# eridgd/WCT-TF

Hardware: AMD Instinct MI355X
Metric: stylized frames/sec @512x512, 5-level relu5->1 pipeline, alpha=0.8 (higher is better)
Workload: dtype f16

## Files before the change

### wct_tf_amd/csrc/conv_wino.hip

```cpp
#include "common.h"

namespace {
typedef unsigned int u32x4 __attribute__((ext_vector_type(4)));
typedef _Float16 h2 __attribute__((ext_vector_type(2)));
constexpr int TW = 16;
constexpr int PITCH = 20;
constexpr int BK = 32;

__device__ __forceinline__ half8 pk_sub(half8 a, half8 b) {
  u32x4 ua = __builtin_bit_cast(u32x4, a), ub = __builtin_bit_cast(u32x4, b), r;
#pragma unroll
  for (int i = 0; i < 4; ++i) {
    unsigned o;
    asm("v_pk_add_f16 %0, %1, %2 neg_lo:[0,1] neg_hi:[0,1]" : "=v"(o) : "v"(ua[i]), "v"(ub[i]));
    r[i] = o;
  }
  return __builtin_bit_cast(half8, r);
}

__device__ __forceinline__ int reflect_idx(int i, int n) {
  if (i < 0) i = -i;
  if (i >= n) i = 2 * n - 2 - i;
  i = i < 0 ? 0 : i;
  return i >= n ? n - 1 : i;
}

template <int TH, int BN, int WM, int WN, bool IL>
__global__ __launch_bounds__(256, TH >= 16 ? 1 : 2)
void conv3x3_wino_kernel(ConvArgs p, int tiles_x, int n_tiles) {
  constexpr int PR = TH / 2;
  constexpr int MT = (PR / 2) / WM;
  constexpr int NT = (BN / 32) / WN;
  constexpr int G = 256 / PR;
  constexpr int SL = (72 + G - 1) / G;
  constexpr int PATCH_BYTES = PR * 4 * PITCH * 64;
  constexpr int DUMP_OFF = 2 * PATCH_BYTES;
  constexpr int PF_TAP = 5;
  static_assert(PR % 2 == 0 && (PR / 2) % WM == 0 && 256 % PR == 0 && WM * WN == 4, "tile shape");

  extern __shared__ __attribute__((aligned(16))) unsigned char smem[];
  const int tid = threadIdx.x, lane = tid & 63, wave = tid >> 6;
  const int wm = wave / WN, wn = wave % WN;
  int bid = blockIdx.x;
  const int ntile = bid % n_tiles;
  bid /= n_tiles;
  const int tx = bid % tiles_x, ty = bid / tiles_x;
  const int b = blockIdx.y;
  const int y0 = ty * TH, x0 = tx * TW, n0 = ntile * BN;

  const int Hin = p.upsample ? p.H / 2 : p.H;
  const int Win = p.upsample ? p.W / 2 : p.W;
  const half_t* xb = p.x + (size_t)b * Hin * Win * p.Cin;
  const __amdgpu_buffer_rsrc_t w_rsrc = __builtin_amdgcn_make_buffer_rsrc((void*)p.w_wino, 0, 0x7FFFFFFF, 0x00020000);
  const __amdgpu_buffer_rsrc_t x_rsrc = __builtin_amdgcn_make_buffer_rsrc((void*)xb, 0, 0x7FFFFFFF, 0x00020000);

  const int lpr = tid / G, ls = tid % G;
  unsigned row_off[4], col_off[SL], dst_off[SL];
  bool slot_ok[SL];
#pragma unroll
  for (int i = 0; i < 4; ++i) {
    int iy = reflect_idx(y0 + 2 * lpr - 1 + i, p.H);
    if (p.upsample) iy >>= 1;
    row_off[i] = (unsigned)(iy * Win) * p.Cin * 2;
  }
#pragma unroll
  for (int j = 0; j < SL; ++j) {
    const int slot = ls + j * G;
    slot_ok[j] = slot < 72;
    const int px = slot_ok[j] ? slot >> 2 : 0, piece = slot & 3;
    int ix = reflect_idx(x0 - 1 + px, p.W);
    if (p.upsample) ix >>= 1;
    col_off[j] = (unsigned)(ix * p.Cin + piece * 8) * 2;
    dst_off[j] = ((lpr * 4 * PITCH + px) * 4 + (piece ^ ((px >> 2) & 3))) * 16;
    if (IL && !slot_ok[j]) dst_off[j] = DUMP_OFF + tid * 16;
  }
  u32x4 raw[SL][4];
  auto load_rows = [&](int chunk) {
#pragma unroll
    for (int j = 0; j < SL; ++j)
#pragma unroll
      for (int i = 0; i < 4; ++i)
        raw[j][i] = __builtin_amdgcn_raw_buffer_load_b128(x_rsrc, row_off[i] + col_off[j], chunk * BK * 2, 0);
  };
  auto park_rows = [&](int buf) {
#pragma unroll
    for (int j = 0; j < SL; ++j) {
      const half8 d0 = __builtin_bit_cast(half8, raw[j][0]), d1 = __builtin_bit_cast(half8, raw[j][1]);
      const half8 d2 = __builtin_bit_cast(half8, raw[j][2]), d3 = __builtin_bit_cast(half8, raw[j][3]);
      const half8 t0 = pk_sub(d0, d2), t1 = d1 + d2, t2 = pk_sub(d2, d1), t3 = pk_sub(d1, d3);
      if (slot_ok[j]) {
        unsigned char* d = smem + buf * PATCH_BYTES + dst_off[j];
        *reinterpret_cast<half8*>(d) = t0;
        *reinterpret_cast<half8*>(d + PITCH * 64) = t1;
        *reinterpret_cast<half8*>(d + 2 * PITCH * 64) = t2;
        *reinterpret_cast<half8*>(d + 3 * PITCH * 64) = t3;
      }
    }
  };

  const int frag_px = lane & 15, frag_pr = (lane & 31) >> 4, kgrp = lane >> 5;
  int rd_base[3][2];
#pragma unroll
  for (int kx = 0; kx < 3; ++kx)
#pragma unroll
    for (int ks = 0; ks < 2; ++ks) {
      const int px = frag_px + kx;
      rd_base[kx][ks] = (((wm * MT * 2 + frag_pr) * 4) * PITCH + px) * 64 + (((ks * 2 + kgrp) ^ ((px >> 2) & 3)) * 16);
    }
  const int c16 = p.Cin >> 4;
  unsigned wfrag[NT];
#pragma unroll
  for (int nt = 0; nt < NT; ++nt) wfrag[nt] = (((n0 >> 5) + wn * NT + nt) * 12 * c16 * 512 + lane * 8) * 2;

  f32x16 acc[4][NT][MT];
#pragma unroll
  for (int nt = 0; nt < NT; ++nt) {
    f32x4 bv[4];
#pragma unroll
    for (int rq = 0; rq < 4; ++rq) bv[rq] = *reinterpret_cast<const f32x4*>(p.bias + n0 + (wn * NT + nt) * 32 + 8 * rq + 4 * kgrp);
#pragma unroll
    for (int f = 0; f < 4; ++f)
#pragma unroll
      for (int mt = 0; mt < MT; ++mt)
#pragma unroll
        for (int r = 0; r < 16; ++r) acc[f][nt][mt][r] = f == 1 ? bv[r >> 2][r & 3] : 0.f;
  }

  const int n_chunks = p.Cin / BK;
  half8 wf[3][NT][2];
  half8 bf[IL ? 3 : 2][2][MT];
  auto load_w = [&](half8 (&dst)[NT][2], int tap12, int chunk) {
    const int soff = (tap12 * c16 + chunk * 2) * 1024;
#pragma unroll
    for (int nt = 0; nt < NT; ++nt)
#pragma unroll
      for (int ks = 0; ks < 2; ++ks)
        dst[nt][ks] = __builtin_bit_cast(half8, __builtin_amdgcn_raw_buffer_load_b128(w_rsrc, wfrag[nt] + ks * 1024, soff, 0));
  };
  auto read_b = [&](half8 (&dst)[2][MT], int f, int kx, int buf) {
#pragma unroll
    for (int ks = 0; ks < 2; ++ks)
#pragma unroll
      for (int mt = 0; mt < MT; ++mt)
        dst[ks][mt] = *reinterpret_cast<const half8*>(smem + buf * PATCH_BYTES + rd_base[kx][ks] + (mt * 8 + f) * PITCH * 64);
  };

  if constexpr (IL) {
    constexpr int NM = 2 * MT * NT;
    constexpr int NR = 2 * NT + 2 * MT;
#ifndef WINO_LT0
#define WINO_LT0 1
#define WINO_PT0 6
#endif
    constexpr int LT0 = WINO_LT0, PT0 = WINO_PT0;
    static_assert(LT0 + SL <= PT0 && PT0 + SL <= 10, "staging schedule");
#ifndef WINO_WRING
#define WINO_WRING 4
#endif
#ifndef WINO_ABL
#define WINO_ABL 0
#endif
#ifndef WINO_RAW_AUX
#define WINO_RAW_AUX 0
#endif
    constexpr int ABL = WINO_ABL;
    constexpr int WR = WINO_WRING, WA = WR - 1;
    static_assert(24 % WR == 0, "ring");
    half8 wq[WR][NT][2];
    half8 tq[4];
    load_rows(0);
#pragma unroll
    for (int i = 0; i < WA; ++i) load_w(wq[i], i, 0);
#pragma unroll
    for (int j = 0; j < SL; ++j) {
      const half8 d0 = __builtin_bit_cast(half8, raw[j][0]), d1 = __builtin_bit_cast(half8, raw[j][1]);
      const half8 d2 = __builtin_bit_cast(half8, raw[j][2]), d3 = __builtin_bit_cast(half8, raw[j][3]);
      unsigned char* d = smem + dst_off[j];
      *reinterpret_cast<half8*>(d) = pk_sub(d0, d2);
      *reinterpret_cast<half8*>(d + PITCH * 64) = d1 + d2;
      *reinterpret_cast<half8*>(d + 2 * PITCH * 64) = pk_sub(d2, d1);
      *reinterpret_cast<half8*>(d + 3 * PITCH * 64) = pk_sub(d1, d3);
    }
    asm volatile("s_waitcnt lgkmcnt(0)\n\ts_barrier" ::: "memory");
    read_b(bf[0], 0, 0, 0);
    read_b(bf[1], 0, 1, 0);
#pragma unroll 1
    for (int pair = 0; pair < n_chunks; pair += 2) {
#pragma unroll
      for (int t = 0; t < 24; ++t) {
        const int tt = t % 12, chunk_i = pair + t / 12, buf = t / 12;
        const int f = tt / 3, kx = tt % 3;
        const int chunk_n = chunk_i + 1 < n_chunks ? chunk_i + 1 : chunk_i;
        const int t3 = (tt + WA) % 12, c3 = tt + WA >= 12 ? chunk_n : chunk_i;
        const int t1 = (tt + 2) % 12, buf1 = tt >= 10 ? buf ^ 1 : buf;
        const int soff3 = (t3 * c16 + c3 * 2) * 1024;
#pragma unroll
        for (int j = 0; j < NM; ++j) {
          const int ks = j / (MT * NT), mt = (j / NT) % MT, nt = j % NT;
          if (!(ABL & 4)) acc[f][nt][mt] = __builtin_amdgcn_mfma_f32_32x32x16_f16(wq[t % WR][nt][ks], bf[t % 3][ks][mt], acc[f][nt][mt], 0, 0, 0);
          else asm volatile("" :: "v"(wq[t % WR][nt][ks]), "v"(bf[t % 3][ks][mt]));
#pragma unroll
          for (int k = j * NR / NM; k < (j + 1) * NR / NM; ++k) {
            if (k < 2 * NT) {
              if (!(ABL & 1)) wq[(t + WA) % WR][k / 2][k % 2] =
                  __builtin_bit_cast(half8, __builtin_amdgcn_raw_buffer_load_b128(w_rsrc, wfrag[k / 2] + (k % 2) * 1024, soff3, 0));
            } else {
              const int kk = k - 2 * NT, ks1 = kk / MT, mt1 = kk % MT;
              if (!(ABL & 8)) bf[(t + 2) % 3][ks1][mt1] = *reinterpret_cast<const half8*>(smem + buf1 * PATCH_BYTES + rd_base[t1 % 3][ks1] + (mt1 * 8 + t1 / 3) * PITCH * 64);
            }
          }
          if (tt >= LT0 && tt < LT0 + SL) {
            const int sl = tt - LT0;
            if (j < 4 && !(ABL & 2)) raw[sl][j] = __builtin_amdgcn_raw_buffer_load_b128(x_rsrc, (ABL & 64) ? (lane & 3) * 16 + j * 64 + sl * 256 : row_off[j] + col_off[sl], (ABL & 32) ? 0 : chunk_n * BK * 2, WINO_RAW_AUX);
          }
          if (tt >= PT0 && tt < PT0 + SL && !(ABL & 16)) {
            const int sl = tt - PT0;
            {
#pragma unroll
              for (int it = j * 8 / NM; it < (j + 1) * 8 / NM; ++it) {
                const int fq = it >> 1;
                if ((it & 1) == 0) {
                  const half8 da = __builtin_bit_cast(half8, raw[sl][fq == 0 ? 0 : fq == 1 ? 1 : fq == 2 ? 2 : 1]);
                  const half8 db = __builtin_bit_cast(half8, raw[sl][fq == 0 ? 2 : fq == 1 ? 2 : fq == 2 ? 1 : 3]);
                  tq[fq] = fq == 1 ? da + db : pk_sub(da, db);
                } else {
                  *reinterpret_cast<half8*>(smem + (buf ^ 1) * PATCH_BYTES * (slot_ok[sl] ? 1 : 0) + dst_off[sl] + fq * PITCH * 64) = tq[fq];
                }
              }
            }
          }
          __builtin_amdgcn_sched_barrier(0);
        }
        if (tt == 9) asm volatile("s_waitcnt lgkmcnt(0)\n\ts_barrier" ::: "memory");
      }
    }
  } else {
  load_rows(0);
  load_w(wf[0], 0, 0);
  load_w(wf[1], 1, 0);
  park_rows(0);
  asm volatile("s_waitcnt lgkmcnt(0)\n\ts_barrier" ::: "memory");
  read_b(bf[0], 0, 0, 0);

#pragma unroll 1
  for (int pair = 0; pair < n_chunks; pair += 2) {
#pragma unroll
    for (int t = 0; t < 24; ++t) {
      const int tt = t % 12, chunk_i = pair + t / 12, buf = t / 12;
      const int f = tt / 3, kx = tt % 3;
      const bool more = chunk_i + 1 < n_chunks;
      {
        const int t2 = (tt + 2) % 12;
        const int c2 = tt + 2 >= 12 ? (more ? chunk_i + 1 : chunk_i) : chunk_i;
        load_w(wf[(t + 2) % 3], t2, c2);
      }
      if (tt == PF_TAP && more) load_rows(chunk_i + 1);
      if (tt != 11) read_b(bf[(t + 1) & 1], (tt + 1) / 3, (tt + 1) % 3, buf);
      else if (more) read_b(bf[(t + 1) & 1], 0, 0, buf ^ 1);
      __builtin_amdgcn_sched_barrier(0);
#pragma unroll
      for (int ks = 0; ks < 2; ++ks)
#pragma unroll
        for (int mt = 0; mt < MT; ++mt)
#pragma unroll
          for (int nt = 0; nt < NT; ++nt)
            acc[f][nt][mt] = __builtin_amdgcn_mfma_f32_32x32x16_f16(wf[t % 3][nt][ks], bf[t & 1][ks][mt], acc[f][nt][mt], 0, 0, 0);
      __builtin_amdgcn_sched_barrier(0);
      if (tt == 10 && more) {
        park_rows(buf ^ 1);
        asm volatile("s_waitcnt lgkmcnt(0)\n\ts_barrier" ::: "memory");
      }
    }
  }

  }
  constexpr int OOB = (int)0x80000000u;
  const int Ho = p.pool ? (p.H + 1) / 2 : p.H, Wo = p.pool ? (p.W + 1) / 2 : p.W;
  const unsigned img_elems = (unsigned)Ho * Wo * p.Cout;
  const __amdgpu_buffer_rsrc_t r16 = __builtin_amdgcn_make_buffer_rsrc((void*)(p.y16 + (size_t)b * img_elems), 0, img_elems * 2, 0x00020000);
  const float lo1 = p.relu ? 0.f : -__builtin_inff();
  const h2 lo2 = {(half_t)lo1, (half_t)lo1};
  const h2 zero2 = {(half_t)0.f, (half_t)0.f};
  const int ox = x0 + frag_px;
  const int chan = n0 + wn * NT * 32;
#pragma unroll
  for (int mt = 0; mt < MT; ++mt) {
    const int oy = y0 + ((wm * MT + mt) * 2 + frag_pr) * 2;
    const bool in0 = (oy < p.H) & (ox < p.W), in1 = (oy + 1 < p.H) & (ox < p.W);
    int off[2];
    if (p.pool) {
      off[0] = in0 && (frag_px & 1) == 0 ? (((oy >> 1) * Wo + (ox >> 1)) * p.Cout + chan + 8 * kgrp) * 2 : OOB;
      off[1] = OOB;
    } else {
      off[0] = in0 ? ((oy * p.W + ox) * p.Cout + chan + 8 * kgrp) * 2 : OOB;
      off[1] = in1 ? (((oy + 1) * p.W + ox) * p.Cout + chan + 8 * kgrp) * 2 : OOB;
    }
#pragma unroll
    for (int nt = 0; nt < NT; ++nt) {
      unsigned pk[2][4][2];
#pragma unroll
      for (int rq = 0; rq < 4; ++rq) {
        f32x4 e, o;
#pragma unroll
        for (int j = 0; j < 4; ++j) {
          const int r = rq * 4 + j;
          const float m0 = acc[0][nt][mt][r], m1 = acc[1][nt][mt][r], m2 = acc[2][nt][mt][r], m3 = acc[3][nt][mt][r];
          e[j] = (m0 + m1) + m2;
          o[j] = (m1 - m2) - m3;
        }
        h2 e0 = {(half_t)e[0], (half_t)e[1]}, e1 = {(half_t)e[2], (half_t)e[3]};
        h2 o0 = {(half_t)o[0], (half_t)o[1]}, o1 = {(half_t)o[2], (half_t)o[3]};
        e0 = __builtin_elementwise_max(e0, lo2); e1 = __builtin_elementwise_max(e1, lo2);
        o0 = __builtin_elementwise_max(o0, lo2); o1 = __builtin_elementwise_max(o1, lo2);
        if (p.pool) {
          h2 q[2] = {__builtin_elementwise_max(in0 ? e0 : zero2, in1 ? o0 : zero2), __builtin_elementwise_max(in0 ? e1 : zero2, in1 ? o1 : zero2)};
#pragma unroll
          for (int d = 0; d < 2; ++d) {
            const unsigned tq = __builtin_bit_cast(unsigned, q[d]);
            const h2 nb = __builtin_bit_cast(h2, __builtin_amdgcn_update_dpp(0, (int)tq, 0xB1, 0xF, 0xF, true));
            q[d] = __builtin_elementwise_max(q[d], nb);
          }
          e0 = q[0]; e1 = q[1];
        }
        pk[0][rq][0] = __builtin_bit_cast(unsigned, e0); pk[0][rq][1] = __builtin_bit_cast(unsigned, e1);
        pk[1][rq][0] = __builtin_bit_cast(unsigned, o0); pk[1][rq][1] = __builtin_bit_cast(unsigned, o1);
      }
#pragma unroll
      for (int par = 0; par < 2; ++par) {
#pragma unroll
        for (int m = 0; m < 2; ++m) {
          auto sx = __builtin_amdgcn_permlane32_swap(pk[par][2 * m][0], pk[par][2 * m + 1][0], false, false);
          auto sy = __builtin_amdgcn_permlane32_swap(pk[par][2 * m][1], pk[par][2 * m + 1][1], false, false);
          u32x4 ov = {sx[0], sy[0], sx[1], sy[1]};
          __builtin_amdgcn_raw_buffer_store_b128(ov, r16, off[par] + (nt * 32 + 16 * m) * 2, 0, 0);
        }
      }
    }
  }
}

template <int TH, int BN, int WM, int WN, bool IL = false>
int launch_wino_cfg(const ConvArgs& a, hipStream_t s) {
  const int tiles_x = cdiv(a.W, TW), tiles_y = cdiv(a.H, TH), n_tiles = a.Cout / BN;
  const size_t lds = 2 * (size_t)(TH / 2) * 4 * PITCH * 64 + (IL ? 8192 : 0);
  HIP_TRY(hipFuncSetAttribute(reinterpret_cast<const void*>(&conv3x3_wino_kernel<TH, BN, WM, WN, IL>),
                              hipFuncAttributeMaxDynamicSharedMemorySize, (int)lds));
  hipLaunchKernelGGL((conv3x3_wino_kernel<TH, BN, WM, WN, IL>), dim3(tiles_x * tiles_y * n_tiles, a.B), dim3(256), lds, s, a, tiles_x, n_tiles);
  HIP_TRY(hipGetLastError());
  return WCT_OK;
}
}

bool conv3x3_wino_takes(const ConvArgs& a) {
  return a.w_wino != nullptr && a.y16 != nullptr && a.y32 == nullptr && a.usum == nullptr && a.img1 == nullptr &&
         a.Cin % 64 == 0 && a.Cout % 64 == 0 && (!a.pool || a.relu);
}

int launch_conv3x3_wino(const ConvArgs& a, hipStream_t s) {
  ARG_CHECK(conv3x3_wino_takes(a) && a.H > 1 && a.W > 1 && a.B > 0);
  ARG_CHECK(!a.upsample || (a.H % 2 == 0 && a.W % 2 == 0));
  ARG_CHECK((size_t)a.H * a.W * a.Cin * 2 < ((size_t)1 << 31));
  ARG_CHECK((size_t)a.H * a.W * a.Cout * 2 < ((size_t)1 << 31));
  const long px16 = (long)cdiv(a.W, TW) * cdiv(a.H, 16) * a.B;
  const long px8 = (long)cdiv(a.W, TW) * cdiv(a.H, 8) * a.B;
  if (a.Cout % 128 == 0 && px16 * (a.Cout / 128) >= 256) return launch_wino_cfg<16, 128, 1, 4, true>(a, s);
  if (a.Cout % 128 == 0 && px8 * (a.Cout / 128) >= 256) return launch_wino_cfg<8, 128, 1, 4>(a, s);
  return launch_wino_cfg<8, 64, 2, 2>(a, s);
}
```

Before: 684.2.

## Specialize Winograd conv for nearest-upsampled input to use three row transforms

Adds a compile-time UP variant of the Winograd F(2,3) conv kernel for inputs that were nearest-neighbour upsampled. Paired output rows then share duplicated source rows, so one input-transform row is zero and the kernel keeps only three transformed rows (9 taps instead of 12), with weight taps remapped. This cuts MFMA work, LDS footprint and input loads for the decoder's upsample convs. The cost is a rescheduled pipeline (ring size, staging taps) tuned only for the new tap count, and row clamping in place of reflection, which changes border semantics and relies on the tile start y0 being even.

New measurement: 685.3 (median of 6 runs). No clear change (+0.2%).

```diff
diff --git a/wct_tf_amd/csrc/conv_wino.hip b/wct_tf_amd/csrc/conv_wino.hip
--- a/wct_tf_amd/csrc/conv_wino.hip
+++ b/wct_tf_amd/csrc/conv_wino.hip
@@ -25,17 +25,20 @@
   return i >= n ? n - 1 : i;
 }
 
-template <int TH, int BN, int WM, int WN, bool IL>
+template <int TH, int BN, int WM, int WN, bool IL, bool UP>
 __global__ __launch_bounds__(256, TH >= 16 ? 1 : 2)
 void conv3x3_wino_kernel(ConvArgs p, int tiles_x, int n_tiles) {
+  constexpr int NF = UP ? 3 : 4;
+  constexpr int NTAP = NF * 3;
+  auto wtap = [](int t) { return (UP && t >= 6 ? t + 3 : t); };
   constexpr int PR = TH / 2;
   constexpr int MT = (PR / 2) / WM;
   constexpr int NT = (BN / 32) / WN;
   constexpr int G = 256 / PR;
   constexpr int SL = (72 + G - 1) / G;
-  constexpr int PATCH_BYTES = PR * 4 * PITCH * 64;
+  constexpr int PATCH_BYTES = PR * NF * PITCH * 64;
   constexpr int DUMP_OFF = 2 * PATCH_BYTES;
-  constexpr int PF_TAP = 5;
+  constexpr int PF_TAP = NTAP - 7;
   static_assert(PR % 2 == 0 && (PR / 2) % WM == 0 && 256 % PR == 0 && WM * WN == 4, "tile shape");
 
   extern __shared__ __attribute__((aligned(16))) unsigned char smem[];
@@ -48,19 +51,25 @@
   const int b = blockIdx.y;
   const int y0 = ty * TH, x0 = tx * TW, n0 = ntile * BN;
 
-  const int Hin = p.upsample ? p.H / 2 : p.H;
-  const int Win = p.upsample ? p.W / 2 : p.W;
+  const int Hin = UP ? p.H / 2 : p.H;
+  const int Win = UP ? p.W / 2 : p.W;
   const half_t* xb = p.x + (size_t)b * Hin * Win * p.Cin;
   const __amdgpu_buffer_rsrc_t w_rsrc = __builtin_amdgcn_make_buffer_rsrc((void*)p.w_wino, 0, 0x7FFFFFFF, 0x00020000);
   const __amdgpu_buffer_rsrc_t x_rsrc = __builtin_amdgcn_make_buffer_rsrc((void*)xb, 0, 0x7FFFFFFF, 0x00020000);
 
   const int lpr = tid / G, ls = tid % G;
-  unsigned row_off[4], col_off[SL], dst_off[SL];
+  unsigned row_off[NF], col_off[SL], dst_off[SL];
   bool slot_ok[SL];
 #pragma unroll
-  for (int i = 0; i < 4; ++i) {
-    int iy = reflect_idx(y0 + 2 * lpr - 1 + i, p.H);
-    if (p.upsample) iy >>= 1;
+  for (int i = 0; i < NF; ++i) {
+    int iy;
+    if constexpr (UP) {
+      iy = (y0 >> 1) + lpr - 1 + i;
+      iy = iy < 0 ? 0 : iy;
+      iy = iy >= Hin ? Hin - 1 : iy;
+    } else {
+      iy = reflect_idx(y0 + 2 * lpr - 1 + i, p.H);
+    }
     row_off[i] = (unsigned)(iy * Win) * p.Cin * 2;
   }
 #pragma unroll
@@ -69,31 +78,35 @@
     slot_ok[j] = slot < 72;
     const int px = slot_ok[j] ? slot >> 2 : 0, piece = slot & 3;
     int ix = reflect_idx(x0 - 1 + px, p.W);
-    if (p.upsample) ix >>= 1;
+    if (UP) ix >>= 1;
     col_off[j] = (unsigned)(ix * p.Cin + piece * 8) * 2;
-    dst_off[j] = ((lpr * 4 * PITCH + px) * 4 + (piece ^ ((px >> 2) & 3))) * 16;
+    dst_off[j] = ((lpr * NF * PITCH + px) * 4 + (piece ^ ((px >> 2) & 3))) * 16;
     if (IL && !slot_ok[j]) dst_off[j] = DUMP_OFF + tid * 16;
   }
-  u32x4 raw[SL][4];
+  u32x4 raw[SL][NF];
   auto load_rows = [&](int chunk) {
 #pragma unroll
     for (int j = 0; j < SL; ++j)
 #pragma unroll
-      for (int i = 0; i < 4; ++i)
+      for (int i = 0; i < NF; ++i)
         raw[j][i] = __builtin_amdgcn_raw_buffer_load_b128(x_rsrc, row_off[i] + col_off[j], chunk * BK * 2, 0);
   };
+  auto piece = [&](const u32x4 (&r)[NF], int q) {
+    const int ia = UP ? (q == 0 ? 0 : 1) : (q == 0 ? 0 : q == 1 ? 1 : q == 2 ? 2 : 1);
+    const int ib = UP ? (q == 0 ? 1 : q == 1 ? 1 : 2) : (q == 0 ? 2 : q == 1 ? 2 : q == 2 ? 1 : 3);
+    const half8 da = __builtin_bit_cast(half8, r[ia]), db = __builtin_bit_cast(half8, r[ib]);
+    return q == 1 ? da + db : pk_sub(da, db);
+  };
   auto park_rows = [&](int buf) {
 #pragma unroll
     for (int j = 0; j < SL; ++j) {
-      const half8 d0 = __builtin_bit_cast(half8, raw[j][0]), d1 = __builtin_bit_cast(half8, raw[j][1]);
-      const half8 d2 = __builtin_bit_cast(half8, raw[j][2]), d3 = __builtin_bit_cast(half8, raw[j][3]);
-      const half8 t0 = pk_sub(d0, d2), t1 = d1 + d2, t2 = pk_sub(d2, d1), t3 = pk_sub(d1, d3);
+      half8 t[NF];
+#pragma unroll
+      for (int q = 0; q < NF; ++q) t[q] = piece(raw[j], q);
       if (slot_ok[j]) {
         unsigned char* d = smem + buf * PATCH_BYTES + dst_off[j];
-        *reinterpret_cast<half8*>(d) = t0;
-        *reinterpret_cast<half8*>(d + PITCH * 64) = t1;
-        *reinterpret_cast<half8*>(d + 2 * PITCH * 64) = t2;
-        *reinterpret_cast<half8*>(d + 3 * PITCH * 64) = t3;
+#pragma unroll
+        for (int q = 0; q < NF; ++q) *reinterpret_cast<half8*>(d + q * PITCH * 64) = t[q];
       }
     }
   };
@@ -105,21 +118,21 @@
 #pragma unroll
     for (int ks = 0; ks < 2; ++ks) {
       const int px = frag_px + kx;
-      rd_base[kx][ks] = (((wm * MT * 2 + frag_pr) * 4) * PITCH + px) * 64 + (((ks * 2 + kgrp) ^ ((px >> 2) & 3)) * 16);
+      rd_base[kx][ks] = (((wm * MT * 2 + frag_pr) * NF) * PITCH + px) * 64 + (((ks * 2 + kgrp) ^ ((px >> 2) & 3)) * 16);
     }
   const int c16 = p.Cin >> 4;
   unsigned wfrag[NT];
 #pragma unroll
   for (int nt = 0; nt < NT; ++nt) wfrag[nt] = (((n0 >> 5) + wn * NT + nt) * 12 * c16 * 512 + lane * 8) * 2;
 
-  f32x16 acc[4][NT][MT];
+  f32x16 acc[NF][NT][MT];
 #pragma unroll
   for (int nt = 0; nt < NT; ++nt) {
     f32x4 bv[4];
 #pragma unroll
     for (int rq = 0; rq < 4; ++rq) bv[rq] = *reinterpret_cast<const f32x4*>(p.bias + n0 + (wn * NT + nt) * 32 + 8 * rq + 4 * kgrp);
 #pragma unroll
-    for (int f = 0; f < 4; ++f)
+    for (int f = 0; f < NF; ++f)
 #pragma unroll
       for (int mt = 0; mt < MT; ++mt)
 #pragma unroll
@@ -129,8 +142,8 @@
   const int n_chunks = p.Cin / BK;
   half8 wf[3][NT][2];
   half8 bf[IL ? 3 : 2][2][MT];
-  auto load_w = [&](half8 (&dst)[NT][2], int tap12, int chunk) {
-    const int soff = (tap12 * c16 + chunk * 2) * 1024;
+  auto load_w = [&](half8 (&dst)[NT][2], int tap, int chunk) {
+    const int soff = (wtap(tap) * c16 + chunk * 2) * 1024;
 #pragma unroll
     for (int nt = 0; nt < NT; ++nt)
 #pragma unroll
@@ -142,7 +155,7 @@
     for (int ks = 0; ks < 2; ++ks)
 #pragma unroll
       for (int mt = 0; mt < MT; ++mt)
-        dst[ks][mt] = *reinterpret_cast<const half8*>(smem + buf * PATCH_BYTES + rd_base[kx][ks] + (mt * 8 + f) * PITCH * 64);
+        dst[ks][mt] = *reinterpret_cast<const half8*>(smem + buf * PATCH_BYTES + rd_base[kx][ks] + (mt * 2 * NF + f) * PITCH * 64);
   };
 
   if constexpr (IL) {
@@ -152,8 +165,8 @@
 #define WINO_LT0 1
 #define WINO_PT0 6
 #endif
-    constexpr int LT0 = WINO_LT0, PT0 = WINO_PT0;
-    static_assert(LT0 + SL <= PT0 && PT0 + SL <= 10, "staging schedule");
+    constexpr int LT0 = UP ? 0 : WINO_LT0, PT0 = UP ? 4 : WINO_PT0;
+    static_assert(LT0 + SL <= PT0 && PT0 + SL <= NTAP - 2, "staging schedule");
 #ifndef WINO_WRING
 #define WINO_WRING 4
 #endif
@@ -164,22 +177,18 @@
 #define WINO_RAW_AUX 0
 #endif
     constexpr int ABL = WINO_ABL;
-    constexpr int WR = WINO_WRING, WA = WR - 1;
-    static_assert(24 % WR == 0, "ring");
+    constexpr int WR = UP ? 6 : WINO_WRING, WA = WR - 1;
+    static_assert((2 * NTAP) % WR == 0 && WA < NTAP, "ring");
     half8 wq[WR][NT][2];
-    half8 tq[4];
+    half8 tq[NF];
     load_rows(0);
 #pragma unroll
     for (int i = 0; i < WA; ++i) load_w(wq[i], i, 0);
 #pragma unroll
     for (int j = 0; j < SL; ++j) {
-      const half8 d0 = __builtin_bit_cast(half8, raw[j][0]), d1 = __builtin_bit_cast(half8, raw[j][1]);
-      const half8 d2 = __builtin_bit_cast(half8, raw[j][2]), d3 = __builtin_bit_cast(half8, raw[j][3]);
       unsigned char* d = smem + dst_off[j];
-      *reinterpret_cast<half8*>(d) = pk_sub(d0, d2);
-      *reinterpret_cast<half8*>(d + PITCH * 64) = d1 + d2;
-      *reinterpret_cast<half8*>(d + 2 * PITCH * 64) = pk_sub(d2, d1);
-      *reinterpret_cast<half8*>(d + 3 * PITCH * 64) = pk_sub(d1, d3);
+#pragma unroll
+      for (int q = 0; q < NF; ++q) *reinterpret_cast<half8*>(d + q * PITCH * 64) = piece(raw[j], q);
     }
     asm volatile("s_waitcnt lgkmcnt(0)\n\ts_barrier" ::: "memory");
     read_b(bf[0], 0, 0, 0);
@@ -187,13 +196,13 @@
 #pragma unroll 1
     for (int pair = 0; pair < n_chunks; pair += 2) {
 #pragma unroll
-      for (int t = 0; t < 24; ++t) {
-        const int tt = t % 12, chunk_i = pair + t / 12, buf = t / 12;
-        const int f = tt / 3, kx = tt % 3;
+      for (int t = 0; t < 2 * NTAP; ++t) {
+        const int tt = t % NTAP, chunk_i = pair + t / NTAP, buf = t / NTAP;
+        const int f = tt / 3;
         const int chunk_n = chunk_i + 1 < n_chunks ? chunk_i + 1 : chunk_i;
-        const int t3 = (tt + WA) % 12, c3 = tt + WA >= 12 ? chunk_n : chunk_i;
-        const int t1 = (tt + 2) % 12, buf1 = tt >= 10 ? buf ^ 1 : buf;
-        const int soff3 = (t3 * c16 + c3 * 2) * 1024;
+        const int t3 = (tt + WA) % NTAP, c3 = tt + WA >= NTAP ? chunk_n : chunk_i;
+        const int t1 = (tt + 2) % NTAP, buf1 = tt >= NTAP - 2 ? buf ^ 1 : buf;
+        const int soff3 = (wtap(t3) * c16 + c3 * 2) * 1024;
 #pragma unroll
         for (int j = 0; j < NM; ++j) {
           const int ks = j / (MT * NT), mt = (j / NT) % MT, nt = j % NT;
@@ -206,23 +215,21 @@
                   __builtin_bit_cast(half8, __builtin_amdgcn_raw_buffer_load_b128(w_rsrc, wfrag[k / 2] + (k % 2) * 1024, soff3, 0));
             } else {
               const int kk = k - 2 * NT, ks1 = kk / MT, mt1 = kk % MT;
-              if (!(ABL & 8)) bf[(t + 2) % 3][ks1][mt1] = *reinterpret_cast<const half8*>(smem + buf1 * PATCH_BYTES + rd_base[t1 % 3][ks1] + (mt1 * 8 + t1 / 3) * PITCH * 64);
+              if (!(ABL & 8)) bf[(t + 2) % 3][ks1][mt1] = *reinterpret_cast<const half8*>(smem + buf1 * PATCH_BYTES + rd_base[t1 % 3][ks1] + (mt1 * 2 * NF + t1 / 3) * PITCH * 64);
             }
           }
           if (tt >= LT0 && tt < LT0 + SL) {
             const int sl = tt - LT0;
-            if (j < 4 && !(ABL & 2)) raw[sl][j] = __builtin_amdgcn_raw_buffer_load_b128(x_rsrc, (ABL & 64) ? (lane & 3) * 16 + j * 64 + sl * 256 : row_off[j] + col_off[sl], (ABL & 32) ? 0 : chunk_n * BK * 2, WINO_RAW_AUX);
+            if (j < NF && !(ABL & 2)) raw[sl][j] = __builtin_amdgcn_raw_buffer_load_b128(x_rsrc, (ABL & 64) ? (lane & 3) * 16 + j * 64 + sl * 256 : row_off[j] + col_off[sl], (ABL & 32) ? 0 : chunk_n * BK * 2, WINO_RAW_AUX);
           }
           if (tt >= PT0 && tt < PT0 + SL && !(ABL & 16)) {
             const int sl = tt - PT0;
             {
 #pragma unroll
-              for (int it = j * 8 / NM; it < (j + 1) * 8 / NM; ++it) {
+              for (int it = j * 2 * NF / NM; it < (j + 1) * 2 * NF / NM; ++it) {
                 const int fq = it >> 1;
                 if ((it & 1) == 0) {
-                  const half8 da = __builtin_bit_cast(half8, raw[sl][fq == 0 ? 0 : fq == 1 ? 1 : fq == 2 ? 2 : 1]);
-                  const half8 db = __builtin_bit_cast(half8, raw[sl][fq == 0 ? 2 : fq == 1 ? 2 : fq == 2 ? 1 : 3]);
-                  tq[fq] = fq == 1 ? da + db : pk_sub(da, db);
+                  tq[fq] = piece(raw[sl], fq);
                 } else {
                   *reinterpret_cast<half8*>(smem + (buf ^ 1) * PATCH_BYTES * (slot_ok[sl] ? 1 : 0) + dst_off[sl] + fq * PITCH * 64) = tq[fq];
                 }
@@ -231,7 +238,7 @@
           }
           __builtin_amdgcn_sched_barrier(0);
         }
-        if (tt == 9) asm volatile("s_waitcnt lgkmcnt(0)\n\ts_barrier" ::: "memory");
+        if (tt == NTAP - 3) asm volatile("s_waitcnt lgkmcnt(0)\n\ts_barrier" ::: "memory");
       }
     }
   } else {
@@ -245,17 +252,17 @@
 #pragma unroll 1
   for (int pair = 0; pair < n_chunks; pair += 2) {
 #pragma unroll
-    for (int t = 0; t < 24; ++t) {
-      const int tt = t % 12, chunk_i = pair + t / 12, buf = t / 12;
-      const int f = tt / 3, kx = tt % 3;
+    for (int t = 0; t < 2 * NTAP; ++t) {
+      const int tt = t % NTAP, chunk_i = pair + t / NTAP, buf = t / NTAP;
+      const int f = tt / 3;
       const bool more = chunk_i + 1 < n_chunks;
       {
-        const int t2 = (tt + 2) % 12;
-        const int c2 = tt + 2 >= 12 ? (more ? chunk_i + 1 : chunk_i) : chunk_i;
+        const int t2 = (tt + 2) % NTAP;
+        const int c2 = tt + 2 >= NTAP ? (more ? chunk_i + 1 : chunk_i) : chunk_i;
         load_w(wf[(t + 2) % 3], t2, c2);
       }
       if (tt == PF_TAP && more) load_rows(chunk_i + 1);
-      if (tt != 11) read_b(bf[(t + 1) & 1], (tt + 1) / 3, (tt + 1) % 3, buf);
+      if (tt != NTAP - 1) read_b(bf[(t + 1) & 1], (tt + 1) / 3, (tt + 1) % 3, buf);
       else if (more) read_b(bf[(t + 1) & 1], 0, 0, buf ^ 1);
       __builtin_amdgcn_sched_barrier(0);
 #pragma unroll
@@ -266,7 +273,7 @@
           for (int nt = 0; nt < NT; ++nt)
             acc[f][nt][mt] = __builtin_amdgcn_mfma_f32_32x32x16_f16(wf[t % 3][nt][ks], bf[t & 1][ks][mt], acc[f][nt][mt], 0, 0, 0);
       __builtin_amdgcn_sched_barrier(0);
-      if (tt == 10 && more) {
+      if (tt == NTAP - 2 && more) {
         park_rows(buf ^ 1);
         asm volatile("s_waitcnt lgkmcnt(0)\n\ts_barrier" ::: "memory");
       }
@@ -304,7 +311,7 @@
 #pragma unroll
         for (int j = 0; j < 4; ++j) {
           const int r = rq * 4 + j;
-          const float m0 = acc[0][nt][mt][r], m1 = acc[1][nt][mt][r], m2 = acc[2][nt][mt][r], m3 = acc[3][nt][mt][r];
+          const float m0 = acc[0][nt][mt][r], m1 = acc[1][nt][mt][r], m2 = UP ? 0.0f : acc[2][nt][mt][r], m3 = acc[NF - 1][nt][mt][r];
           e[j] = (m0 + m1) + m2;
           o[j] = (m1 - m2) - m3;
         }
@@ -339,15 +346,20 @@
   }
 }
 
+template <int TH, int BN, int WM, int WN, bool IL, bool UP>
+int launch_wino_up(const ConvArgs& a, hipStream_t s) {
+  const int tiles_x = cdiv(a.W, TW), tiles_y = cdiv(a.H, TH), n_tiles = a.Cout / BN;
+  const size_t lds = 2 * (size_t)(TH / 2) * (UP ? 3 : 4) * PITCH * 64 + (IL ? 8192 : 0);
+  HIP_TRY(hipFuncSetAttribute(reinterpret_cast<const void*>(&conv3x3_wino_kernel<TH, BN, WM, WN, IL, UP>),
+                              hipFuncAttributeMaxDynamicSharedMemorySize, (int)lds));
+  hipLaunchKernelGGL((conv3x3_wino_kernel<TH, BN, WM, WN, IL, UP>), dim3(tiles_x * tiles_y * n_tiles, a.B), dim3(256), lds, s, a, tiles_x, n_tiles);
+  HIP_TRY(hipGetLastError());
+  return WCT_OK;
+}
+
 template <int TH, int BN, int WM, int WN, bool IL = false>
 int launch_wino_cfg(const ConvArgs& a, hipStream_t s) {
-  const int tiles_x = cdiv(a.W, TW), tiles_y = cdiv(a.H, TH), n_tiles = a.Cout / BN;
-  const size_t lds = 2 * (size_t)(TH / 2) * 4 * PITCH * 64 + (IL ? 8192 : 0);
-  HIP_TRY(hipFuncSetAttribute(reinterpret_cast<const void*>(&conv3x3_wino_kernel<TH, BN, WM, WN, IL>),
-                              hipFuncAttributeMaxDynamicSharedMemorySize, (int)lds));
-  hipLaunchKernelGGL((conv3x3_wino_kernel<TH, BN, WM, WN, IL>), dim3(tiles_x * tiles_y * n_tiles, a.B), dim3(256), lds, s, a, tiles_x, n_tiles);
-  HIP_TRY(hipGetLastError());
-  return WCT_OK;
+  return a.upsample ? launch_wino_up<TH, BN, WM, WN, IL, true>(a, s) : launch_wino_up<TH, BN, WM, WN, IL, false>(a, s);
 }
 }
 
```

## Specialize Winograd conv for nearest-upsampled input using three row transforms

Applied to the files above, without the earlier changes.

Adds an UP template variant for convolutions whose input is a nearest-neighbour 2x upsample. Because adjacent input rows repeat, one of the four Winograd row-transform terms is zero, so the kernel keeps three row pieces. This cuts LDS patch size, global row loads, MFMA taps (9 instead of 12 per chunk) and accumulator registers, and skips the corresponding weight taps. The staging schedule and weight ring are retuned for the shorter tap loop, which carries a risk of correctness errors in the index remapping.

Measured after the change: 667.0 before, 670.5 after (median of 6 runs). About the same (+0.5%).

```diff
diff --git a/wct_tf_amd/csrc/conv_wino.hip b/wct_tf_amd/csrc/conv_wino.hip
--- a/wct_tf_amd/csrc/conv_wino.hip
+++ b/wct_tf_amd/csrc/conv_wino.hip
@@ -25,7 +25,7 @@
   return i >= n ? n - 1 : i;
 }
 
-template <int TH, int BN, int WM, int WN, bool IL>
+template <int TH, int BN, int WM, int WN, bool IL, bool UP>
 __global__ __launch_bounds__(256, TH >= 16 ? 1 : 2)
 void conv3x3_wino_kernel(ConvArgs p, int tiles_x, int n_tiles) {
   constexpr int PR = TH / 2;
@@ -33,9 +33,11 @@
   constexpr int NT = (BN / 32) / WN;
   constexpr int G = 256 / PR;
   constexpr int SL = (72 + G - 1) / G;
-  constexpr int PATCH_BYTES = PR * 4 * PITCH * 64;
+  constexpr int NF = UP ? 3 : 4;
+  constexpr int NTAP = NF * 3;
+  constexpr int PATCH_BYTES = PR * NF * PITCH * 64;
   constexpr int DUMP_OFF = 2 * PATCH_BYTES;
-  constexpr int PF_TAP = 5;
+  constexpr int PF_TAP = UP ? 3 : 5;
   static_assert(PR % 2 == 0 && (PR / 2) % WM == 0 && 256 % PR == 0 && WM * WN == 4, "tile shape");
 
   extern __shared__ __attribute__((aligned(16))) unsigned char smem[];
@@ -55,11 +57,11 @@
   const __amdgpu_buffer_rsrc_t x_rsrc = __builtin_amdgcn_make_buffer_rsrc((void*)xb, 0, 0x7FFFFFFF, 0x00020000);
 
   const int lpr = tid / G, ls = tid % G;
-  unsigned row_off[4], col_off[SL], dst_off[SL];
+  unsigned row_off[NF], col_off[SL], dst_off[SL];
   bool slot_ok[SL];
 #pragma unroll
-  for (int i = 0; i < 4; ++i) {
-    int iy = reflect_idx(y0 + 2 * lpr - 1 + i, p.H);
+  for (int i = 0; i < NF; ++i) {
+    int iy = reflect_idx(y0 + 2 * lpr - 1 + (UP && i == 2 ? 3 : i), p.H);
     if (p.upsample) iy >>= 1;
     row_off[i] = (unsigned)(iy * Win) * p.Cin * 2;
   }
@@ -71,29 +73,33 @@
     int ix = reflect_idx(x0 - 1 + px, p.W);
     if (p.upsample) ix >>= 1;
     col_off[j] = (unsigned)(ix * p.Cin + piece * 8) * 2;
-    dst_off[j] = ((lpr * 4 * PITCH + px) * 4 + (piece ^ ((px >> 2) & 3))) * 16;
+    dst_off[j] = ((lpr * NF * PITCH + px) * 4 + (piece ^ ((px >> 2) & 3))) * 16;
     if (IL && !slot_ok[j]) dst_off[j] = DUMP_OFF + tid * 16;
   }
-  u32x4 raw[SL][4];
+  u32x4 raw[SL][NF];
   auto load_rows = [&](int chunk) {
 #pragma unroll
     for (int j = 0; j < SL; ++j)
 #pragma unroll
-      for (int i = 0; i < 4; ++i)
+      for (int i = 0; i < NF; ++i)
         raw[j][i] = __builtin_amdgcn_raw_buffer_load_b128(x_rsrc, row_off[i] + col_off[j], chunk * BK * 2, 0);
   };
+  auto piece = [&](const u32x4 (&r)[NF], int i) {
+    const int a = UP ? (i == 0 ? 0 : 1) : (i == 0 ? 0 : i == 1 ? 1 : i == 2 ? 2 : 1);
+    const int b = UP ? (i == 0 ? 1 : i == 1 ? 1 : 2) : (i == 0 ? 2 : i == 1 ? 2 : i == 2 ? 1 : 3);
+    const half8 da = __builtin_bit_cast(half8, r[a]), db = __builtin_bit_cast(half8, r[b]);
+    return i == 1 ? da + db : pk_sub(da, db);
+  };
   auto park_rows = [&](int buf) {
 #pragma unroll
     for (int j = 0; j < SL; ++j) {
-      const half8 d0 = __builtin_bit_cast(half8, raw[j][0]), d1 = __builtin_bit_cast(half8, raw[j][1]);
-      const half8 d2 = __builtin_bit_cast(half8, raw[j][2]), d3 = __builtin_bit_cast(half8, raw[j][3]);
-      const half8 t0 = pk_sub(d0, d2), t1 = d1 + d2, t2 = pk_sub(d2, d1), t3 = pk_sub(d1, d3);
+      half8 t[NF];
+#pragma unroll
+      for (int i = 0; i < NF; ++i) t[i] = piece(raw[j], i);
       if (slot_ok[j]) {
         unsigned char* d = smem + buf * PATCH_BYTES + dst_off[j];
-        *reinterpret_cast<half8*>(d) = t0;
-        *reinterpret_cast<half8*>(d + PITCH * 64) = t1;
-        *reinterpret_cast<half8*>(d + 2 * PITCH * 64) = t2;
-        *reinterpret_cast<half8*>(d + 3 * PITCH * 64) = t3;
+#pragma unroll
+        for (int i = 0; i < NF; ++i) *reinterpret_cast<half8*>(d + i * PITCH * 64) = t[i];
       }
     }
   };
@@ -105,21 +111,21 @@
 #pragma unroll
     for (int ks = 0; ks < 2; ++ks) {
       const int px = frag_px + kx;
-      rd_base[kx][ks] = (((wm * MT * 2 + frag_pr) * 4) * PITCH + px) * 64 + (((ks * 2 + kgrp) ^ ((px >> 2) & 3)) * 16);
+      rd_base[kx][ks] = (((wm * MT * 2 + frag_pr) * NF) * PITCH + px) * 64 + (((ks * 2 + kgrp) ^ ((px >> 2) & 3)) * 16);
     }
   const int c16 = p.Cin >> 4;
   unsigned wfrag[NT];
 #pragma unroll
   for (int nt = 0; nt < NT; ++nt) wfrag[nt] = (((n0 >> 5) + wn * NT + nt) * 12 * c16 * 512 + lane * 8) * 2;
 
-  f32x16 acc[4][NT][MT];
+  f32x16 acc[NF][NT][MT];
 #pragma unroll
   for (int nt = 0; nt < NT; ++nt) {
     f32x4 bv[4];
 #pragma unroll
     for (int rq = 0; rq < 4; ++rq) bv[rq] = *reinterpret_cast<const f32x4*>(p.bias + n0 + (wn * NT + nt) * 32 + 8 * rq + 4 * kgrp);
 #pragma unroll
-    for (int f = 0; f < 4; ++f)
+    for (int f = 0; f < NF; ++f)
 #pragma unroll
       for (int mt = 0; mt < MT; ++mt)
 #pragma unroll
@@ -129,8 +135,9 @@
   const int n_chunks = p.Cin / BK;
   half8 wf[3][NT][2];
   half8 bf[IL ? 3 : 2][2][MT];
-  auto load_w = [&](half8 (&dst)[NT][2], int tap12, int chunk) {
-    const int soff = (tap12 * c16 + chunk * 2) * 1024;
+  auto wtap = [](int tap) { return UP && tap >= 6 ? tap + 3 : tap; };
+  auto load_w = [&](half8 (&dst)[NT][2], int tap, int chunk) {
+    const int soff = (wtap(tap) * c16 + chunk * 2) * 1024;
 #pragma unroll
     for (int nt = 0; nt < NT; ++nt)
 #pragma unroll
@@ -142,7 +149,7 @@
     for (int ks = 0; ks < 2; ++ks)
 #pragma unroll
       for (int mt = 0; mt < MT; ++mt)
-        dst[ks][mt] = *reinterpret_cast<const half8*>(smem + buf * PATCH_BYTES + rd_base[kx][ks] + (mt * 8 + f) * PITCH * 64);
+        dst[ks][mt] = *reinterpret_cast<const half8*>(smem + buf * PATCH_BYTES + rd_base[kx][ks] + (mt * 2 * NF + f) * PITCH * 64);
   };
 
   if constexpr (IL) {
@@ -152,11 +159,18 @@
 #define WINO_LT0 1
 #define WINO_PT0 6
 #endif
-    constexpr int LT0 = WINO_LT0, PT0 = WINO_PT0;
-    static_assert(LT0 + SL <= PT0 && PT0 + SL <= 10, "staging schedule");
+#ifndef WINO_UP_LT0
+#define WINO_UP_LT0 1
+#define WINO_UP_PT0 4
+#endif
+    constexpr int LT0 = UP ? WINO_UP_LT0 : WINO_LT0, PT0 = UP ? WINO_UP_PT0 : WINO_PT0;
+    static_assert(LT0 >= 0 && LT0 + SL <= PT0 && PT0 + SL <= NTAP - 2, "staging schedule");
 #ifndef WINO_WRING
 #define WINO_WRING 4
 #endif
+#ifndef WINO_UP_WRING
+#define WINO_UP_WRING 6
+#endif
 #ifndef WINO_ABL
 #define WINO_ABL 0
 #endif
@@ -164,22 +178,18 @@
 #define WINO_RAW_AUX 0
 #endif
     constexpr int ABL = WINO_ABL;
-    constexpr int WR = WINO_WRING, WA = WR - 1;
-    static_assert(24 % WR == 0, "ring");
+    constexpr int WR = UP ? WINO_UP_WRING : WINO_WRING, WA = WR - 1;
+    static_assert((2 * NTAP) % WR == 0 && (2 * NTAP) % 3 == 0 && WA < NTAP, "ring");
     half8 wq[WR][NT][2];
-    half8 tq[4];
+    half8 tq[NF];
     load_rows(0);
 #pragma unroll
     for (int i = 0; i < WA; ++i) load_w(wq[i], i, 0);
 #pragma unroll
     for (int j = 0; j < SL; ++j) {
-      const half8 d0 = __builtin_bit_cast(half8, raw[j][0]), d1 = __builtin_bit_cast(half8, raw[j][1]);
-      const half8 d2 = __builtin_bit_cast(half8, raw[j][2]), d3 = __builtin_bit_cast(half8, raw[j][3]);
       unsigned char* d = smem + dst_off[j];
-      *reinterpret_cast<half8*>(d) = pk_sub(d0, d2);
-      *reinterpret_cast<half8*>(d + PITCH * 64) = d1 + d2;
-      *reinterpret_cast<half8*>(d + 2 * PITCH * 64) = pk_sub(d2, d1);
-      *reinterpret_cast<half8*>(d + 3 * PITCH * 64) = pk_sub(d1, d3);
+#pragma unroll
+      for (int i = 0; i < NF; ++i) *reinterpret_cast<half8*>(d + i * PITCH * 64) = piece(raw[j], i);
     }
     asm volatile("s_waitcnt lgkmcnt(0)\n\ts_barrier" ::: "memory");
     read_b(bf[0], 0, 0, 0);
@@ -187,13 +197,13 @@
 #pragma unroll 1
     for (int pair = 0; pair < n_chunks; pair += 2) {
 #pragma unroll
-      for (int t = 0; t < 24; ++t) {
-        const int tt = t % 12, chunk_i = pair + t / 12, buf = t / 12;
-        const int f = tt / 3, kx = tt % 3;
+      for (int t = 0; t < 2 * NTAP; ++t) {
+        const int tt = t % NTAP, chunk_i = pair + t / NTAP, buf = t / NTAP;
+        const int f = tt / 3;
         const int chunk_n = chunk_i + 1 < n_chunks ? chunk_i + 1 : chunk_i;
-        const int t3 = (tt + WA) % 12, c3 = tt + WA >= 12 ? chunk_n : chunk_i;
-        const int t1 = (tt + 2) % 12, buf1 = tt >= 10 ? buf ^ 1 : buf;
-        const int soff3 = (t3 * c16 + c3 * 2) * 1024;
+        const int t3 = (tt + WA) % NTAP, c3 = tt + WA >= NTAP ? chunk_n : chunk_i;
+        const int t1 = (tt + 2) % NTAP, buf1 = tt >= NTAP - 2 ? buf ^ 1 : buf;
+        const int soff3 = (wtap(t3) * c16 + c3 * 2) * 1024;
 #pragma unroll
         for (int j = 0; j < NM; ++j) {
           const int ks = j / (MT * NT), mt = (j / NT) % MT, nt = j % NT;
@@ -206,23 +216,21 @@
                   __builtin_bit_cast(half8, __builtin_amdgcn_raw_buffer_load_b128(w_rsrc, wfrag[k / 2] + (k % 2) * 1024, soff3, 0));
             } else {
               const int kk = k - 2 * NT, ks1 = kk / MT, mt1 = kk % MT;
-              if (!(ABL & 8)) bf[(t + 2) % 3][ks1][mt1] = *reinterpret_cast<const half8*>(smem + buf1 * PATCH_BYTES + rd_base[t1 % 3][ks1] + (mt1 * 8 + t1 / 3) * PITCH * 64);
+              if (!(ABL & 8)) bf[(t + 2) % 3][ks1][mt1] = *reinterpret_cast<const half8*>(smem + buf1 * PATCH_BYTES + rd_base[t1 % 3][ks1] + (mt1 * 2 * NF + t1 / 3) * PITCH * 64);
             }
           }
           if (tt >= LT0 && tt < LT0 + SL) {
             const int sl = tt - LT0;
-            if (j < 4 && !(ABL & 2)) raw[sl][j] = __builtin_amdgcn_raw_buffer_load_b128(x_rsrc, (ABL & 64) ? (lane & 3) * 16 + j * 64 + sl * 256 : row_off[j] + col_off[sl], (ABL & 32) ? 0 : chunk_n * BK * 2, WINO_RAW_AUX);
+            if (j < NF && !(ABL & 2)) raw[sl][j] = __builtin_amdgcn_raw_buffer_load_b128(x_rsrc, (ABL & 64) ? (lane & 3) * 16 + j * 64 + sl * 256 : row_off[j] + col_off[sl], (ABL & 32) ? 0 : chunk_n * BK * 2, WINO_RAW_AUX);
           }
           if (tt >= PT0 && tt < PT0 + SL && !(ABL & 16)) {
             const int sl = tt - PT0;
             {
 #pragma unroll
-              for (int it = j * 8 / NM; it < (j + 1) * 8 / NM; ++it) {
+              for (int it = j * 2 * NF / NM; it < (j + 1) * 2 * NF / NM; ++it) {
                 const int fq = it >> 1;
                 if ((it & 1) == 0) {
-                  const half8 da = __builtin_bit_cast(half8, raw[sl][fq == 0 ? 0 : fq == 1 ? 1 : fq == 2 ? 2 : 1]);
-                  const half8 db = __builtin_bit_cast(half8, raw[sl][fq == 0 ? 2 : fq == 1 ? 2 : fq == 2 ? 1 : 3]);
-                  tq[fq] = fq == 1 ? da + db : pk_sub(da, db);
+                  tq[fq] = piece(raw[sl], fq);
                 } else {
                   *reinterpret_cast<half8*>(smem + (buf ^ 1) * PATCH_BYTES * (slot_ok[sl] ? 1 : 0) + dst_off[sl] + fq * PITCH * 64) = tq[fq];
                 }
@@ -231,7 +239,7 @@
           }
           __builtin_amdgcn_sched_barrier(0);
         }
-        if (tt == 9) asm volatile("s_waitcnt lgkmcnt(0)\n\ts_barrier" ::: "memory");
+        if (tt == NTAP - 3) asm volatile("s_waitcnt lgkmcnt(0)\n\ts_barrier" ::: "memory");
       }
     }
   } else {
@@ -245,17 +253,17 @@
 #pragma unroll 1
   for (int pair = 0; pair < n_chunks; pair += 2) {
 #pragma unroll
-    for (int t = 0; t < 24; ++t) {
-      const int tt = t % 12, chunk_i = pair + t / 12, buf = t / 12;
-      const int f = tt / 3, kx = tt % 3;
+    for (int t = 0; t < 2 * NTAP; ++t) {
+      const int tt = t % NTAP, chunk_i = pair + t / NTAP, buf = t / NTAP;
+      const int f = tt / 3;
       const bool more = chunk_i + 1 < n_chunks;
       {
-        const int t2 = (tt + 2) % 12;
-        const int c2 = tt + 2 >= 12 ? (more ? chunk_i + 1 : chunk_i) : chunk_i;
+        const int t2 = (tt + 2) % NTAP;
+        const int c2 = tt + 2 >= NTAP ? (more ? chunk_i + 1 : chunk_i) : chunk_i;
         load_w(wf[(t + 2) % 3], t2, c2);
       }
       if (tt == PF_TAP && more) load_rows(chunk_i + 1);
-      if (tt != 11) read_b(bf[(t + 1) & 1], (tt + 1) / 3, (tt + 1) % 3, buf);
+      if (tt != NTAP - 1) read_b(bf[(t + 1) & 1], (tt + 1) / 3, (tt + 1) % 3, buf);
       else if (more) read_b(bf[(t + 1) & 1], 0, 0, buf ^ 1);
       __builtin_amdgcn_sched_barrier(0);
 #pragma unroll
@@ -266,7 +274,7 @@
           for (int nt = 0; nt < NT; ++nt)
             acc[f][nt][mt] = __builtin_amdgcn_mfma_f32_32x32x16_f16(wf[t % 3][nt][ks], bf[t & 1][ks][mt], acc[f][nt][mt], 0, 0, 0);
       __builtin_amdgcn_sched_barrier(0);
-      if (tt == 10 && more) {
+      if (tt == NTAP - 2 && more) {
         park_rows(buf ^ 1);
         asm volatile("s_waitcnt lgkmcnt(0)\n\ts_barrier" ::: "memory");
       }
@@ -304,7 +312,7 @@
 #pragma unroll
         for (int j = 0; j < 4; ++j) {
           const int r = rq * 4 + j;
-          const float m0 = acc[0][nt][mt][r], m1 = acc[1][nt][mt][r], m2 = acc[2][nt][mt][r], m3 = acc[3][nt][mt][r];
+          const float m0 = acc[0][nt][mt][r], m1 = acc[1][nt][mt][r], m2 = UP ? 0.f : acc[2][nt][mt][r], m3 = acc[NF - 1][nt][mt][r];
           e[j] = (m0 + m1) + m2;
           o[j] = (m1 - m2) - m3;
         }
@@ -339,15 +347,20 @@
   }
 }
 
+template <int TH, int BN, int WM, int WN, bool IL, bool UP>
+int launch_wino_variant(const ConvArgs& a, hipStream_t s) {
+  const int tiles_x = cdiv(a.W, TW), tiles_y = cdiv(a.H, TH), n_tiles = a.Cout / BN;
+  const size_t lds = 2 * (size_t)(TH / 2) * (UP ? 3 : 4) * PITCH * 64 + (IL ? 8192 : 0);
+  HIP_TRY(hipFuncSetAttribute(reinterpret_cast<const void*>(&conv3x3_wino_kernel<TH, BN, WM, WN, IL, UP>),
+                              hipFuncAttributeMaxDynamicSharedMemorySize, (int)lds));
+  hipLaunchKernelGGL((conv3x3_wino_kernel<TH, BN, WM, WN, IL, UP>), dim3(tiles_x * tiles_y * n_tiles, a.B), dim3(256), lds, s, a, tiles_x, n_tiles);
+  HIP_TRY(hipGetLastError());
+  return WCT_OK;
+}
+
 template <int TH, int BN, int WM, int WN, bool IL = false>
 int launch_wino_cfg(const ConvArgs& a, hipStream_t s) {
-  const int tiles_x = cdiv(a.W, TW), tiles_y = cdiv(a.H, TH), n_tiles = a.Cout / BN;
-  const size_t lds = 2 * (size_t)(TH / 2) * 4 * PITCH * 64 + (IL ? 8192 : 0);
-  HIP_TRY(hipFuncSetAttribute(reinterpret_cast<const void*>(&conv3x3_wino_kernel<TH, BN, WM, WN, IL>),
-                              hipFuncAttributeMaxDynamicSharedMemorySize, (int)lds));
-  hipLaunchKernelGGL((conv3x3_wino_kernel<TH, BN, WM, WN, IL>), dim3(tiles_x * tiles_y * n_tiles, a.B), dim3(256), lds, s, a, tiles_x, n_tiles);
-  HIP_TRY(hipGetLastError());
-  return WCT_OK;
+  return a.upsample ? launch_wino_variant<TH, BN, WM, WN, IL, true>(a, s) : launch_wino_variant<TH, BN, WM, WN, IL, false>(a, s);
 }
 }
 
```
